# CrispyChillies/Image-Retrieval---Thesis-2026

Hardware: AMD Instinct MI355X
Metric: queries/sec (embed+top-10) over 1M x 1024 gallery (higher is better)
Workload: dtype f32 embed (two fp16 MFMA terms); bf16 MFMA candidates + f64 re-rank

## Files before the change

image-retrieval---thesis-2026_amd/csrc/k_conv3x3_d2h.hip:

```cpp
#include "mirx_device.h"
#include "mirx_kernels.h"

namespace mirx {

namespace {

constexpr int CIN = 128, COUT = 32;
constexpr int KC = 16;
constexpr int NST = CIN / KC;

template <int W, int R, int IPW = 1, int NW = 4>
__global__ __launch_bounds__(64 * NW, NW == 8 ? 1 : 2) void k_conv3x3_d2p(const uint16_t *__restrict__ yt, const uint16_t *__restrict__ w3,
                                                        const float *__restrict__ oscale, float *__restrict__ out,
                                                        int64_t out_bs, const float *__restrict__ in_inv,
                                                        unsigned *__restrict__ out_range, int64_t out_ps, int64_t n_img,
                                                        const float *__restrict__ pool_sc, const float *__restrict__ pool_sh,
                                                        float *__restrict__ pool_out, int64_t pool_bs) {
    constexpr int PW = W + 2, PR = R + 2;
    static_assert(IPW == 1 || R == W, "several images per workgroup: whole images only");
    constexpr int NPIX = IPW * PR * PW;
    constexpr int NP = (NPIX + 31) / 32;
    constexpr int PLANE = NP * 32 * 32;
    constexpr int STAGE = 2 * PLANE;
    constexpr int WSTAGE = 9 * 2 * COUT * KC * 2;
    constexpr int W_LDS0 = 2 * STAGE;
    constexpr int NOUT = IPW * R * W;
    constexpr int NBLK = (NOUT + 31) / 32;
    static_assert(NBLK <= 2 * NW, "two column blocks per wave");
    constexpr int PPW = (2 * NP + NW - 1) / NW;
    constexpr int WPW = (18 + NW - 1) / NW;
    extern __shared__ __attribute__((aligned(16))) char sm[];

    const int wave = __builtin_amdgcn_readfirstlane(threadIdx.x >> 6), lane = threadIdx.x & 63;
    const int half = lane >> 5, n = lane & 31;
    int strip = blockIdx.x;
    int64_t img = blockIdx.y;
    {
        const unsigned nstrip = gridDim.x, lin = blockIdx.x + nstrip * blockIdx.y, full = gridDim.y & ~7u;
        if (lin < nstrip * full) {
            const unsigned j = lin >> 3;
            strip = (int)(j % nstrip);
            img = (int64_t)(j / nstrip) * 8 + (lin & 7);
        }
    }
    const int oy0 = strip * R;
    constexpr unsigned IMG_BYTES = 16u * W * W * 32u;
    img *= IPW;
    const int n_here = (int)(n_img - img < IPW ? n_img - img : IPW);
    const __amdgpu_buffer_rsrc_t yrsrc = __builtin_amdgcn_make_buffer_rsrc((void *)(yt + img * (int64_t)(IMG_BYTES / 2)), 0,
                                                                           (unsigned)n_here * IMG_BYTES, 0x00020000);
    unsigned a_src[PPW];
    int a_dst[PPW];
#pragma unroll
    for (int i = 0; i < PPW; ++i) {
        const int q = wave + NW * i;
        const int term = q / NP, piece = q % NP;
        const int pix = piece * 32 + (lane >> 1);
        const int ji = pix / (PR * PW), prem = pix % (PR * PW);
        const int pr = prem / PW, pc = prem % PW;
        const int iy = oy0 - 1 + pr, ix = pc - 1;
        const bool inside = q < 2 * NP && pix < NPIX && iy >= 0 && iy < W && ix >= 0 && ix < W;
        const int chunk = (lane & 1) ^ ((pix >> 3) & 1);
        a_src[i] = inside ? (unsigned)(ji * IMG_BYTES + (term * W * W + iy * W + ix) * 32 + chunk * 16) : 0xfffffff0u;
        a_dst[i] = q < 2 * NP ? term * PLANE + piece * 1024 : -1;
    }
    auto dma_a = [&](int st, int buf) {
#pragma unroll
        for (int i = 0; i < PPW; ++i)
            if (a_dst[i] >= 0) {
                const unsigned v = a_src[i] == 0xfffffff0u ? a_src[i] : a_src[i] + (unsigned)st * (2u * W * W * 32u);
                __builtin_amdgcn_raw_ptr_buffer_load_lds(yrsrc, LDS_PTR(sm + buf * STAGE + a_dst[i]), 16, v, 0, 0, 0);
            }
    };

    int pbase[2];
    bool live_blk[2];
#pragma unroll
    for (int t = 0; t < 2; ++t) {
        const int blk = wave + NW * t;
        live_blk[t] = blk < NBLK;
        int p = blk * 32 + n;
        if (p >= NOUT) p = NOUT - 1;
        const int pj = p / (R * W), pq = p % (R * W);
        pbase[t] = pj * (PR * PW) + (pq / W) * PW + (pq % W);
    }
    const int a_off = n * 32 + ((half ^ ((n >> 3) & 1)) << 4);
    const __amdgpu_buffer_rsrc_t wrsrc = __builtin_amdgcn_make_buffer_rsrc((void *)w3, 0, NST * WSTAGE, 0x00020000);
    const int w_voff = (lane >> 1) * 32 + (((lane & 1) ^ ((lane >> 4) & 1)) << 4);
    auto dma_w = [&](int st, int buf) {
#pragma unroll
        for (int i = 0; i < WPW; ++i) {
            const int piece = wave + NW * i;
            if (piece < 18)
                __builtin_amdgcn_raw_ptr_buffer_load_lds(wrsrc, LDS_PTR(sm + W_LDS0 + buf * WSTAGE + piece * 1024), 16, w_voff,
                                                         st * WSTAGE + piece * 1024, 0, 0);
        }
    };

    f32x16 acc[2];
#pragma unroll
    for (int t = 0; t < 2; ++t)
#pragma unroll
        for (int r = 0; r < 16; ++r) acc[t][r] = 0.f;

#define MIRX_D2P_READA(DST, TAP)                                                                   \
    {                                                                                              \
        DST[0] = *reinterpret_cast<const f16x8 *>(wb + (2 * (TAP)) * 1024 + a_off);                \
        DST[1] = *reinterpret_cast<const f16x8 *>(wb + (2 * (TAP) + 1) * 1024 + a_off);            \
    }
#define MIRX_D2P_READB(DST, TAP, T)                                                                \
    {                                                                                              \
        const int pix_ = pbase[T] + ((TAP) / 3) * PW + (TAP) % 3;                                  \
        const char *pb_ = sb + pix_ * 32 + ((half ^ ((pix_ >> 3) & 1)) << 4);                      \
        DST[0] = *reinterpret_cast<const f16x8 *>(pb_);                                            \
        DST[1] = *reinterpret_cast<const f16x8 *>(pb_ + PLANE);                                    \
    }
#define MIRX_D2P_MFMA(T, A, B)                                                                     \
    {                                                                                              \
        f32x16 c_ = acc[T];                                                                        \
        c_ = __builtin_amdgcn_mfma_f32_32x32x16_f16(A[1], B[0], c_, 0, 0, 0);                      \
        c_ = __builtin_amdgcn_mfma_f32_32x32x16_f16(A[0], B[1], c_, 0, 0, 0);                      \
        c_ = __builtin_amdgcn_mfma_f32_32x32x16_f16(A[0], B[0], c_, 0, 0, 0);                      \
        acc[T] = c_;                                                                               \
    }
    const bool two = live_blk[1];
    dma_w(0, 0);
    dma_a(0, 0);
    for (int st = 0; st < NST; ++st) {
        const int cur = st & 1;
        asm volatile("s_waitcnt vmcnt(0)" ::: "memory");
        __syncthreads();
        if (st + 1 < NST) {
            dma_w(st + 1, cur ^ 1);
            dma_a(st + 1, cur ^ 1);
        }
        __builtin_amdgcn_sched_barrier(0);
        const char *sb = sm + cur * STAGE;
        const char *wb = sm + W_LDS0 + cur * WSTAGE;
        f16x8 a0[2], a1[2], b0[2], b1[2];
        MIRX_D2P_READA(a0, 0)
        MIRX_D2P_READB(b0, 0, 0)
        if (two) {
#pragma unroll
            for (int tap = 0; tap < 9; ++tap) {
                MIRX_D2P_READB(b1, tap, 1)
                if (tap + 1 < 9) {
                    if (tap & 1) { MIRX_D2P_READA(a0, tap + 1) } else { MIRX_D2P_READA(a1, tap + 1) }
                }
                __builtin_amdgcn_sched_barrier(0);
                if (tap & 1) { MIRX_D2P_MFMA(0, a1, b0) } else { MIRX_D2P_MFMA(0, a0, b0) }
                if (tap + 1 < 9) MIRX_D2P_READB(b0, tap + 1, 0)
                __builtin_amdgcn_sched_barrier(0);
                if (tap & 1) { MIRX_D2P_MFMA(1, a1, b1) } else { MIRX_D2P_MFMA(1, a0, b1) }
            }
        } else {
#pragma unroll
            for (int tap = 0; tap < 9; ++tap) {
                if (tap + 1 < 9) {
                    MIRX_D2P_READB(b1, tap + 1, 0)
                    if (tap & 1) { MIRX_D2P_READA(a0, tap + 1) } else { MIRX_D2P_READA(a1, tap + 1) }
                }
                __builtin_amdgcn_sched_barrier(0);
                if (tap & 1) { MIRX_D2P_MFMA(0, a1, b0) } else { MIRX_D2P_MFMA(0, a0, b0) }
#pragma unroll
                for (int q = 0; q < 2; ++q) b0[q] = b1[q];
            }
        }
    }
#undef MIRX_D2P_READA
#undef MIRX_D2P_READB
#undef MIRX_D2P_MFMA

    float *oi = out + img * out_bs + (int64_t)oy0 * W;
    float osc[16];
#pragma unroll
    for (int r = 0; r < 16; ++r) osc[r] = oscale[8 * (r >> 2) + (r & 3) + 4 * half];
    constexpr int ACT_PITCH = NOUT + 1;
    float *s_act = reinterpret_cast<float *>(sm);
    const bool pooled_twin = IPW == 1 && pool_out != nullptr;
    float psc[16], psh[16];
    if (pooled_twin) {
#pragma unroll
        for (int r = 0; r < 16; ++r) {
            psc[r] = pool_sc[8 * (r >> 2) + (r & 3) + 4 * half];
            psh[r] = pool_sh[8 * (r >> 2) + (r & 3) + 4 * half];
        }
        __syncthreads();
    }
#pragma unroll
    for (int t = 0; t < 2; ++t) {
        const int p = (wave + NW * t) * 32 + n;
        const int pj = p / (R * W), pq = p % (R * W);
        const bool live = live_blk[t] && p < NOUT && pj < n_here && oy0 + pq / W < W;
        const int pimg = (int)img + (pj < n_here ? pj : 0);
        float vmax = 0.f;
        if (live) {
            const float x_inv = in_inv[pimg];
            float *op = oi + (int64_t)pj * out_bs + pq;
#pragma unroll
            for (int r = 0; r < 16; ++r) {
                const int oc = 8 * (r >> 2) + (r & 3) + 4 * half;
                const float v = acc[t][r] * (osc[r] * x_inv);
                vmax = range_max(vmax, v);
                op[(int64_t)oc * out_ps] = v;
                if (pooled_twin) s_act[oc * ACT_PITCH + p] = fmaxf(fmaf(v, psc[r], psh[r]), 0.0f);
            }
        }
        if (out_range && live_blk[t]) {
            if (IPW == 1) range_publish(out_range, (int)img, vmax, lane);
            else range_publish_lanes(out_range, pimg, vmax, lane);
        }
    }
    if constexpr (IPW == 1) {
        if (pooled_twin) {
            __syncthreads();
            constexpr int W2 = W / 2, R2 = R / 2, NP2 = R2 * W2;
            static_assert(R % 2 == 0 && W % 2 == 0, "whole row pairs");
            const int rows_here = W - oy0 < R ? W - oy0 : R;
            float *po = pool_out + img * pool_bs + (int64_t)(oy0 / 2) * W2;
            for (int i = threadIdx.x; i < COUT * NP2; i += 64 * NW) {
                const int oc = i / NP2, q = i % NP2, py = q / W2, px = q % W2;
                if (2 * py < rows_here) {
                    const float *a = s_act + oc * ACT_PITCH + (2 * py) * W + 2 * px;
                    po[(int64_t)oc * (W2 * W2) + q] = (a[0] + a[1] + a[W] + a[W + 1]) * 0.25f;
                }
            }
        }
    }
}

template <int W, int R, int IPW = 1, int NW = 4>
hipError_t launch_d2p(const uint16_t *yt, const uint16_t *w2, const float *oscale, int64_t n, float *out, int64_t out_bs,
                      const float *in_inv, float *out_range, int64_t out_ps, hipStream_t st, const float *pool_sc = nullptr,
                      const float *pool_sh = nullptr, float *pool_out = nullptr, int64_t pool_bs = 0) {
    constexpr int NP = (IPW * (R + 2) * (W + 2) + 31) / 32;
    const size_t lds = (size_t)2 * 2 * NP * 1024 + 2 * 9 * 2 * 32 * 16 * 2;
    static_assert((size_t)2 * 2 * NP * 1024 + 2 * 9 * 2 * 32 * 16 * 2 <= 160 * 1024, "LDS of one CU");
    static std::atomic<unsigned long long> attr_devs{0};
    hipError_t e = set_dynamic_lds(k_conv3x3_d2p<W, R, IPW, NW>, lds, &attr_devs);
    if (e != hipSuccess) return e;
    hipLaunchKernelGGL((k_conv3x3_d2p<W, R, IPW, NW>), dim3((W + R - 1) / R, (unsigned)((n + IPW - 1) / IPW)), dim3(64 * NW), lds,
                       st, yt, w2, oscale, out, out_bs, in_inv, reinterpret_cast<unsigned *>(out_range), out_ps, n, pool_sc, pool_sh,
                       pool_out, pool_bs);
    return hipGetLastError();
}

}

bool conv3x3_takes_small(int64_t n, int side) {
    const int64_t wgs = side == 56 ? 14 * n : side == 28 ? 4 * n : side == 14 ? n : (n + 3) / 4;
    return wgs < conv3x3_small_max_wg();
}

hipError_t launch_conv3x3_d2p(const uint16_t *yt, const uint16_t *w2, const float *oscale, int64_t n, int side, float *out,
                              int64_t out_bs, const float *in_inv, float *out_range, int64_t out_ps, hipStream_t st,
                              const float *pool_sc, const float *pool_sh, float *pool_out, int64_t pool_bs) {
    if (n <= 0) return hipSuccess;
    if (n > 65535 || !in_inv || !oscale) return hipErrorInvalidValue;
    if (!out_ps) out_ps = (int64_t)side * side;
    if (out_ps < (int64_t)side * side) return hipErrorInvalidValue;
    if (pool_out && (!pool_sc || !pool_sh || side == 7 || pool_bs < (int64_t)COUT * (side / 2) * (side / 2)))
        return hipErrorInvalidValue;
    if (conv3x3_takes_small(n, side)) {
        if (pool_out) return hipErrorInvalidValue;
        return launch_conv3x3_d2s(yt, w2, oscale, n, side, out, out_bs, in_inv, out_range, out_ps, st);
    }
#ifndef MIRX_D2P_WAVES
#define MIRX_D2P_WAVES 4
#endif
#if MIRX_D2P_WAVES == 8
    if (pool_out) return hipErrorInvalidValue;
    if (side == 56) return launch_d2p<56, 8, 1, 8>(yt, w2, oscale, n, out, out_bs, in_inv, out_range, out_ps, st);
    if (side == 28) return launch_d2p<28, 14, 1, 8>(yt, w2, oscale, n, out, out_bs, in_inv, out_range, out_ps, st);
    if (side == 14) return launch_d2p<14, 14, 2, 8>(yt, w2, oscale, n, out, out_bs, in_inv, out_range, out_ps, st);
    if (side == 7) return launch_d2p<7, 7, 8, 8>(yt, w2, oscale, n, out, out_bs, in_inv, out_range, out_ps, st);
#else
    if (side == 56) return launch_d2p<56, 4>(yt, w2, oscale, n, out, out_bs, in_inv, out_range, out_ps, st, pool_sc, pool_sh, pool_out, pool_bs);
    if (side == 28) return launch_d2p<28, 8>(yt, w2, oscale, n, out, out_bs, in_inv, out_range, out_ps, st, pool_sc, pool_sh, pool_out, pool_bs);
    if (side == 14) return launch_d2p<14, 14>(yt, w2, oscale, n, out, out_bs, in_inv, out_range, out_ps, st, pool_sc, pool_sh, pool_out, pool_bs);
    if (side == 7) return launch_d2p<7, 7, 4>(yt, w2, oscale, n, out, out_bs, in_inv, out_range, out_ps, st);
#endif
    return hipErrorInvalidValue;
}

}
```

image-retrieval---thesis-2026_amd/csrc/mirx_common.h:

```cpp
#pragma once
#include <hip/hip_runtime.h>
#include <stdint.h>
#include <atomic>
#include <string>

#include "../../include/mirx.h"

#if !defined(MIRX_DIAG) &&                                                                                             \
    (defined(MIRX_EXP_NODMA) || defined(MIRX_EXP_NOBAR) || defined(MIRX_EXP_NOEPI) || defined(MIRX_EXP_NOLDS) ||         \
     defined(MIRX_EXP_SLOTS) || defined(MIRX_EXP_SAMEA) || defined(MIRX_EXP_NOA) || defined(MIRX_EXP_NOB) ||             \
     defined(MIRX_EXP_CYCLES) || defined(MIRX_C1H2_EXP_SKIP) || defined(MIRX_C1H2_EXP_SPLIT) ||                          \
     defined(MIRX_C1H2_EXP_ONE_MFMA) || defined(MIRX_C1H2_STAMPS) || defined(MIRX_LT2_EXP) || defined(MIRX_LH2_EXP) ||   \
     defined(MIRX_DF_EXP) || defined(MIRX_DF_STAMPS) || defined(MIRX_DW_STAMPS) || defined(MIRX_STEM_EXP) ||             \
     defined(MIRX_W3_CYCLES) || defined(MIRX_D2P_WAVES) || defined(MIRX_STEM_PLAIN_ORDER) || defined(MIRX_ATT_EXP))
#error "a MIRX diagnostic switch without -DMIRX_DIAG: these arms give wrong results or alter timing and must never reach libmirx.so"
#endif

namespace mirx {

void set_error(const std::string &msg);
int fail(int code, const std::string &msg);

#define MIRX_HIP(expr)                                                                     \
    do {                                                                                   \
        hipError_t e__ = (expr);                                                           \
        if (e__ != hipSuccess)                                                             \
            return ::mirx::fail(MIRX_EHIP, std::string(#expr) + ": " + hipGetErrorString(e__)); \
    } while (0)

#define MIRX_CHECK(cond, msg)                                   \
    do {                                                        \
        if (!(cond)) return ::mirx::fail(MIRX_EINVAL, (msg));   \
    } while (0)

constexpr int WAVE = 64;
constexpr int DIM_ALIGN = 128;
constexpr int ROW_ALIGN = 256;
constexpr int CAND_CAP = 1024;
constexpr int CAND_OVF = 256;
constexpr int MAX_K = 1024;
constexpr int DEEP_CAP = 4096;
constexpr int DEEP_MIN_SLOTS = 32;
constexpr int DEEP_MAX_REGIONS = 2048;
constexpr int DEEP_TARGET_MUL = 2;
constexpr int DEEP_TARGET_ADD = 512;
constexpr int DEEP_GROUP_ROWS = 512;
constexpr int MAX_DIMP = 4096;

struct Cand {
    float s;
    int32_t row;
};

struct Hit {
    double s;
    int64_t id;
};

__host__ __device__ inline bool hit_before(double sa, int64_t ia, double sb, int64_t ib) {
    return sa > sb || (sa == sb && ia < ib);
}

__host__ __device__ inline uint64_t rank_key(double s) {
    uint64_t u;
    __builtin_memcpy(&u, &s, 8);
    if ((u << 1) == 0) u = 0;
    return (u >> 63) ? u : ~u ^ 0x8000000000000000ull;
}
constexpr uint64_t RANK_KEY_LAST = ~0ull;
constexpr int RANK_TILE = 4096;
constexpr int COMPACT_TILE = 2048;

inline int current_device_cus() {
    static std::atomic<int> cache[64];
    int dev = 0;
    if (hipGetDevice(&dev) != hipSuccess || dev < 0 || dev >= 64) dev = 0;
    int v = cache[dev].load(std::memory_order_relaxed);
    if (v == 0) {
        v = 256;
        (void)hipDeviceGetAttribute(&v, hipDeviceAttributeMultiprocessorCount, dev);
        if (v <= 0) v = 256;
        cache[dev].store(v, std::memory_order_relaxed);
    }
    return v;
}

template <typename Kernel>
inline hipError_t set_dynamic_lds(Kernel *kernel, size_t bytes, std::atomic<unsigned long long> *once = nullptr) {
    int dev = -1;
    if (once && (hipGetDevice(&dev) != hipSuccess || dev < 0 || dev >= 64)) dev = -1;
    if (dev >= 0 && (once->load(std::memory_order_acquire) >> dev & 1ull)) return hipSuccess;
    const hipError_t e = hipFuncSetAttribute(reinterpret_cast<const void *>(kernel), hipFuncAttributeMaxDynamicSharedMemorySize,
                                             (int)bytes);
    if (e == hipSuccess && dev >= 0) once->fetch_or(1ull << dev, std::memory_order_release);
    return e;
}

}
```

Measured before the change: 43950.

## Rebalance d2p DMA pieces across waves and trim work in partial strips

Replaces the round-robin split of weight and activation DMA pieces with a compile-time deal that gives the last wave a lighter share (LIGHT = 20 pieces by default). A static check confirms every piece is issued exactly once. For partial strips or partial image groups, it skips activation loads past the valid pixels and skips MFMA work for empty column blocks. The 8-wave experimental variant is removed. The uneven split changes per-wave issue balance, and the extra per-block bounds logic adds some address arithmetic.

```diff
diff --git a/image-retrieval---thesis-2026_amd/csrc/k_conv3x3_d2h.hip b/image-retrieval---thesis-2026_amd/csrc/k_conv3x3_d2h.hip
--- a/image-retrieval---thesis-2026_amd/csrc/k_conv3x3_d2h.hip
+++ b/image-retrieval---thesis-2026_amd/csrc/k_conv3x3_d2h.hip
@@ -9,8 +9,44 @@
 constexpr int KC = 16;
 constexpr int NST = CIN / KC;
 
-template <int W, int R, int IPW = 1, int NW = 4>
-__global__ __launch_bounds__(64 * NW, NW == 8 ? 1 : 2) void k_conv3x3_d2p(const uint16_t *__restrict__ yt, const uint16_t *__restrict__ w3,
+constexpr int NW = 4;
+#ifndef MIRX_D2P_LIGHT
+#define MIRX_D2P_LIGHT 20
+#endif
+
+template <int NP, int LIGHT>
+struct d2p_deal {
+    static constexpr int NA = 2 * NP, NPIECE = NA + 18;
+    static constexpr int L = LIGHT < 0 ? 0 : LIGHT < NPIECE ? LIGHT : NPIECE;
+    static constexpr int WL = L < 18 ? L : 18, AL = L - WL;
+    static constexpr int NH = LIGHT < 0 ? NW : NW - 1;
+    static constexpr int WH = (18 - WL + NH - 1) / NH, AH = (NA - AL + NH - 1) / NH;
+    static constexpr int WSLOTS = WL > WH ? WL : WH, ASLOTS = AL > AH ? AL : AH;
+    static constexpr bool light(int wave) { return LIGHT >= 0 && wave == NW - 1; }
+    static constexpr int w_piece(int wave, int i) {
+        if (light(wave)) return i < WL ? i : 18;
+        return WL + wave + NH * i;
+    }
+    static constexpr int a_piece(int wave, int i) {
+        if (light(wave)) return i < AL ? i : NA;
+        return AL + (LIGHT < 0 ? wave : (wave + NH - (18 - WL) % NH) % NH) + NH * i;
+    }
+    static constexpr bool partition() {
+        int cnt[NPIECE] = {};
+        for (int wave = 0; wave < NW; ++wave) {
+            for (int i = 0; i < WSLOTS; ++i)
+                if (w_piece(wave, i) < 18) ++cnt[w_piece(wave, i)];
+            for (int i = 0; i < ASLOTS; ++i)
+                if (a_piece(wave, i) < NA) ++cnt[18 + a_piece(wave, i)];
+        }
+        for (int u = 0; u < NPIECE; ++u)
+            if (cnt[u] != 1) return false;
+        return true;
+    }
+};
+
+template <int W, int R, int IPW = 1>
+__global__ __launch_bounds__(64 * NW, 2) void k_conv3x3_d2p(const uint16_t *__restrict__ yt, const uint16_t *__restrict__ w3,
                                                         const float *__restrict__ oscale, float *__restrict__ out,
                                                         int64_t out_bs, const float *__restrict__ in_inv,
                                                         unsigned *__restrict__ out_range, int64_t out_ps, int64_t n_img,
@@ -27,8 +63,10 @@
     constexpr int NOUT = IPW * R * W;
     constexpr int NBLK = (NOUT + 31) / 32;
     static_assert(NBLK <= 2 * NW, "two column blocks per wave");
-    constexpr int PPW = (2 * NP + NW - 1) / NW;
-    constexpr int WPW = (18 + NW - 1) / NW;
+    using deal = d2p_deal<NP, MIRX_D2P_LIGHT>;
+    static_assert(deal::partition(), "every DMA piece of a stage is issued by exactly one wave");
+    constexpr int PPW = deal::ASLOTS;
+    constexpr bool SHORT = IPW > 1 || W % R != 0;
     extern __shared__ __attribute__((aligned(16))) char sm[];
 
     const int wave = __builtin_amdgcn_readfirstlane(threadIdx.x >> 6), lane = threadIdx.x & 63;
@@ -49,11 +87,20 @@
     const int n_here = (int)(n_img - img < IPW ? n_img - img : IPW);
     const __amdgpu_buffer_rsrc_t yrsrc = __builtin_amdgcn_make_buffer_rsrc((void *)(yt + img * (int64_t)(IMG_BYTES / 2)), 0,
                                                                            (unsigned)n_here * IMG_BYTES, 0x00020000);
+    const int rows_here = W - oy0 < R ? W - oy0 : R;
+#if defined(MIRX_D2P_EXP)
+    if (SHORT && (MIRX_D2P_EXP & 1) && (IPW == 1 ? rows_here < R : n_here < IPW)) return;
+    const int nblk_here = (SHORT && (MIRX_D2P_EXP & 2) && (IPW == 1 ? rows_here < R : n_here < IPW)) ? 0 :
+                          !SHORT ? NBLK : ((IPW == 1 ? rows_here * W : n_here * (R * W)) + 31) / 32;
+#else
+    const int nblk_here = !SHORT ? NBLK : ((IPW == 1 ? rows_here * W : n_here * (R * W)) + 31) / 32;
+#endif
+    const int npix_here = !SHORT ? NPIX : IPW == 1 ? (rows_here + 2) * PW : n_here * (PR * PW);
     unsigned a_src[PPW];
     int a_dst[PPW];
 #pragma unroll
     for (int i = 0; i < PPW; ++i) {
-        const int q = wave + NW * i;
+        const int q = deal::a_piece(wave, i);
         const int term = q / NP, piece = q % NP;
         const int pix = piece * 32 + (lane >> 1);
         const int ji = pix / (PR * PW), prem = pix % (PR * PW);
@@ -62,7 +109,7 @@
         const bool inside = q < 2 * NP && pix < NPIX && iy >= 0 && iy < W && ix >= 0 && ix < W;
         const int chunk = (lane & 1) ^ ((pix >> 3) & 1);
         a_src[i] = inside ? (unsigned)(ji * IMG_BYTES + (term * W * W + iy * W + ix) * 32 + chunk * 16) : 0xfffffff0u;
-        a_dst[i] = q < 2 * NP ? term * PLANE + piece * 1024 : -1;
+        a_dst[i] = q < 2 * NP && (!SHORT || piece * 32 < npix_here) ? term * PLANE + piece * 1024 : -1;
     }
     auto dma_a = [&](int st, int buf) {
 #pragma unroll
@@ -78,7 +125,7 @@
 #pragma unroll
     for (int t = 0; t < 2; ++t) {
         const int blk = wave + NW * t;
-        live_blk[t] = blk < NBLK;
+        live_blk[t] = blk < nblk_here;
         int p = blk * 32 + n;
         if (p >= NOUT) p = NOUT - 1;
         const int pj = p / (R * W), pq = p % (R * W);
@@ -88,12 +135,19 @@
     const __amdgpu_buffer_rsrc_t wrsrc = __builtin_amdgcn_make_buffer_rsrc((void *)w3, 0, NST * WSTAGE, 0x00020000);
     const int w_voff = (lane >> 1) * 32 + (((lane & 1) ^ ((lane >> 4) & 1)) << 4);
     auto dma_w = [&](int st, int buf) {
-#pragma unroll
-        for (int i = 0; i < WPW; ++i) {
-            const int piece = wave + NW * i;
-            if (piece < 18)
-                __builtin_amdgcn_raw_ptr_buffer_load_lds(wrsrc, LDS_PTR(sm + W_LDS0 + buf * WSTAGE + piece * 1024), 16, w_voff,
-                                                         st * WSTAGE + piece * 1024, 0, 0);
+        auto issue = [&](int piece) {
+            __builtin_amdgcn_raw_ptr_buffer_load_lds(wrsrc, LDS_PTR(sm + W_LDS0 + buf * WSTAGE + piece * 1024), 16, w_voff,
+                                                     st * WSTAGE + piece * 1024, 0, 0);
+        };
+        if (deal::light(wave)) {
+#pragma unroll
+            for (int i = 0; i < deal::WL; ++i) issue(i);
+        } else {
+#pragma unroll
+            for (int i = 0; i < deal::WH; ++i) {
+                const int piece = deal::w_piece(wave, i);
+                if (piece < 18) issue(piece);
+            }
         }
     };
 
@@ -123,7 +177,7 @@
         c_ = __builtin_amdgcn_mfma_f32_32x32x16_f16(A[0], B[0], c_, 0, 0, 0);                      \
         acc[T] = c_;                                                                               \
     }
-    const bool two = live_blk[1];
+    const bool two = live_blk[1], one = (!SHORT || live_blk[0]) && !two;
     dma_w(0, 0);
     dma_a(0, 0);
     for (int st = 0; st < NST; ++st) {
@@ -153,7 +207,7 @@
                 __builtin_amdgcn_sched_barrier(0);
                 if (tap & 1) { MIRX_D2P_MFMA(1, a1, b1) } else { MIRX_D2P_MFMA(1, a0, b1) }
             }
-        } else {
+        } else if (one) {
 #pragma unroll
             for (int tap = 0; tap < 9; ++tap) {
                 if (tap + 1 < 9) {
@@ -216,7 +270,6 @@
             __syncthreads();
             constexpr int W2 = W / 2, R2 = R / 2, NP2 = R2 * W2;
             static_assert(R % 2 == 0 && W % 2 == 0, "whole row pairs");
-            const int rows_here = W - oy0 < R ? W - oy0 : R;
             float *po = pool_out + img * pool_bs + (int64_t)(oy0 / 2) * W2;
             for (int i = threadIdx.x; i < COUT * NP2; i += 64 * NW) {
                 const int oc = i / NP2, q = i % NP2, py = q / W2, px = q % W2;
@@ -229,7 +282,7 @@
     }
 }
 
-template <int W, int R, int IPW = 1, int NW = 4>
+template <int W, int R, int IPW = 1>
 hipError_t launch_d2p(const uint16_t *yt, const uint16_t *w2, const float *oscale, int64_t n, float *out, int64_t out_bs,
                       const float *in_inv, float *out_range, int64_t out_ps, hipStream_t st, const float *pool_sc = nullptr,
                       const float *pool_sh = nullptr, float *pool_out = nullptr, int64_t pool_bs = 0) {
@@ -237,9 +290,9 @@
     const size_t lds = (size_t)2 * 2 * NP * 1024 + 2 * 9 * 2 * 32 * 16 * 2;
     static_assert((size_t)2 * 2 * NP * 1024 + 2 * 9 * 2 * 32 * 16 * 2 <= 160 * 1024, "LDS of one CU");
     static std::atomic<unsigned long long> attr_devs{0};
-    hipError_t e = set_dynamic_lds(k_conv3x3_d2p<W, R, IPW, NW>, lds, &attr_devs);
+    hipError_t e = set_dynamic_lds(k_conv3x3_d2p<W, R, IPW>, lds, &attr_devs);
     if (e != hipSuccess) return e;
-    hipLaunchKernelGGL((k_conv3x3_d2p<W, R, IPW, NW>), dim3((W + R - 1) / R, (unsigned)((n + IPW - 1) / IPW)), dim3(64 * NW), lds,
+    hipLaunchKernelGGL((k_conv3x3_d2p<W, R, IPW>), dim3((W + R - 1) / R, (unsigned)((n + IPW - 1) / IPW)), dim3(64 * NW), lds,
                        st, yt, w2, oscale, out, out_bs, in_inv, reinterpret_cast<unsigned *>(out_range), out_ps, n, pool_sc, pool_sh,
                        pool_out, pool_bs);
     return hipGetLastError();
@@ -265,21 +318,10 @@
         if (pool_out) return hipErrorInvalidValue;
         return launch_conv3x3_d2s(yt, w2, oscale, n, side, out, out_bs, in_inv, out_range, out_ps, st);
     }
-#ifndef MIRX_D2P_WAVES
-#define MIRX_D2P_WAVES 4
-#endif
-#if MIRX_D2P_WAVES == 8
-    if (pool_out) return hipErrorInvalidValue;
-    if (side == 56) return launch_d2p<56, 8, 1, 8>(yt, w2, oscale, n, out, out_bs, in_inv, out_range, out_ps, st);
-    if (side == 28) return launch_d2p<28, 14, 1, 8>(yt, w2, oscale, n, out, out_bs, in_inv, out_range, out_ps, st);
-    if (side == 14) return launch_d2p<14, 14, 2, 8>(yt, w2, oscale, n, out, out_bs, in_inv, out_range, out_ps, st);
-    if (side == 7) return launch_d2p<7, 7, 8, 8>(yt, w2, oscale, n, out, out_bs, in_inv, out_range, out_ps, st);
-#else
     if (side == 56) return launch_d2p<56, 4>(yt, w2, oscale, n, out, out_bs, in_inv, out_range, out_ps, st, pool_sc, pool_sh, pool_out, pool_bs);
     if (side == 28) return launch_d2p<28, 8>(yt, w2, oscale, n, out, out_bs, in_inv, out_range, out_ps, st, pool_sc, pool_sh, pool_out, pool_bs);
     if (side == 14) return launch_d2p<14, 14>(yt, w2, oscale, n, out, out_bs, in_inv, out_range, out_ps, st, pool_sc, pool_sh, pool_out, pool_bs);
     if (side == 7) return launch_d2p<7, 7, 4>(yt, w2, oscale, n, out, out_bs, in_inv, out_range, out_ps, st);
-#endif
     return hipErrorInvalidValue;
 }
 
diff --git a/image-retrieval---thesis-2026_amd/csrc/mirx_common.h b/image-retrieval---thesis-2026_amd/csrc/mirx_common.h
--- a/image-retrieval---thesis-2026_amd/csrc/mirx_common.h
+++ b/image-retrieval---thesis-2026_amd/csrc/mirx_common.h
@@ -12,7 +12,8 @@
      defined(MIRX_EXP_CYCLES) || defined(MIRX_C1H2_EXP_SKIP) || defined(MIRX_C1H2_EXP_SPLIT) ||                          \
      defined(MIRX_C1H2_EXP_ONE_MFMA) || defined(MIRX_C1H2_STAMPS) || defined(MIRX_LT2_EXP) || defined(MIRX_LH2_EXP) ||   \
      defined(MIRX_DF_EXP) || defined(MIRX_DF_STAMPS) || defined(MIRX_DW_STAMPS) || defined(MIRX_STEM_EXP) ||             \
-     defined(MIRX_W3_CYCLES) || defined(MIRX_D2P_WAVES) || defined(MIRX_STEM_PLAIN_ORDER) || defined(MIRX_ATT_EXP))
+     defined(MIRX_W3_CYCLES) || defined(MIRX_D2P_LIGHT) || defined(MIRX_D2P_EXP) || defined(MIRX_STEM_PLAIN_ORDER) ||    \
+     defined(MIRX_ATT_EXP))
 #error "a MIRX diagnostic switch without -DMIRX_DIAG: these arms give wrong results or alter timing and must never reach libmirx.so"
 #endif
 
```

Result: no change. 44120 (median of 4 runs) (+0.4%).
